# genetics-statistics/GEMMA

Hardware: AMD Instinct MI355X
Metric: SNPs/s (-lmm 1 Wald) at n=20k on 1/2/4/8 MI355X; U^T x HBM GB/s vs roofline (higher is better)
Workload: dtype f64 (U^T x as int8-digit MFMA products with exact int32 accumulation; every column of U scaled by its exact maximum and rounded to 6 base-256 digits = 2^-48 of that maximum -- fp64 keeps 2^-53 per entry; value_strict / strict_leg (7g6m: U^T x at or below the fp64 GEMM's own error) and fp64_gemm_path

## Files before the change

### gemma_amd/_lib.py

```python
import ctypes as C
import os

HERE = os.path.dirname(os.path.abspath(__file__))
LIB_PATH = os.path.join(HERE, "libgemma_hip.so")

SYMBOLS = [
    "gemma_hip_init", "gemma_hip_shutdown", "gemma_hip_abi_version", "gemma_hip_strerror",
    "gemma_hip_last_error", "gemma_hip_device_info", "gemma_hip_dgemm", "gemma_hip_dgemm_d",
    "gemma_hip_kin_begin", "gemma_hip_kin_add", "gemma_hip_kin_add_d", "gemma_hip_kin_end",
    "gemma_hip_kin_end_d", "gemma_hip_kin_loco_d", "gemma_hip_snp_qc", "gemma_hip_center", "gemma_hip_center_d", "gemma_hip_eigh",
    "gemma_hip_eigh_d", "gemma_hip_eigh_reserve", "gemma_hip_eigh_release", "gemma_hip_dbg_eigh_last", "gemma_hip_eigh_sharded_d", "gemma_hip_eigh_kept_K_sharded", "gemma_hip_calc_utx", "gemma_hip_lmm_setup", "gemma_hip_lmm_setup_d",
    "gemma_hip_lmm_null", "gemma_hip_lmm_set_indicator", "gemma_hip_lmm_batch", "gemma_hip_lmm_batch_d",
    "gemma_hip_lmm_assoc_d", "gemma_hip_lmm_finish", "gemma_hip_lm_setup", "gemma_hip_lm_batch", "gemma_hip_lm_batch_d",
    "gemma_hip_lm_finish", "gemma_hip_profile_enable",
    "gemma_hip_profile_read", "gemma_hip_dbg_tridiag", "gemma_hip_dbg_stedc", "gemma_hip_dbg_eigh2", "gemma_hip_dbg_utx", "gemma_hip_lmm_gene_batch", "gemma_hip_lmm_gene_batch_d", "gemma_hip_lmm_set_env",
    "gemma_hip_lmm_gxe_batch", "gemma_hip_lmm_gxe_batch_d",
    "gemma_hip_mvlmm_null", "gemma_hip_mvlmm_set", "gemma_hip_mvlmm_batch", "gemma_hip_mvlmm_batch_d",
    "gemma_hip_kin_end_keep", "gemma_hip_kept_K_get", "gemma_hip_eigh_kept_K", "gemma_hip_eigh_keep", "gemma_hip_kept_n",
    "gemma_hip_kept_bcast", "gemma_hip_kept_U_get", "gemma_hip_calc_utx_kept", "gemma_hip_lmm_setup_kept", "gemma_hip_kept_release",
    "gemma_hip_comm_unique_id", "gemma_hip_comm_init", "gemma_hip_comm_info", "gemma_hip_comm_bcast_d",
    "gemma_hip_comm_allreduce_sum_d", "gemma_hip_comm_finalize", "gemma_hip_comm_selftest", "gemma_hip_comm_stats", "gemma_hip_dbg_i8_digits", "gemma_hip_dbg_last_utx_path", "gemma_hip_lmm_batch_submit", "gemma_hip_lmm_batch_collect",
    "gemma_hip_dbg_last_utx_kernel", "gemma_hip_dbg_last_block_missing", "gemma_hip_dbg_last_i8_post", "gemma_hip_reload_env", "gemma_hip_lmm_batch_pipe_d", "gemma_hip_lmm_pipe_flush",
    "gemma_hip_spd_inverse", "gemma_hip_spd_inverse_d", "gemma_hip_vc_setup", "gemma_hip_vc_setup_d", "gemma_hip_vc_he",
    "gemma_hip_vc_reml", "gemma_hip_vc_timing", "gemma_hip_vc_release",
    "gemma_hip_ridge_setup", "gemma_hip_ridge_setup_d", "gemma_hip_ridge_setup_kept", "gemma_hip_ridge_set_r",
    "gemma_hip_ridge_set_indicator", "gemma_hip_ridge_batch", "gemma_hip_ridge_batch_d", "gemma_hip_ridge_finish",
    "gemma_hip_prdt_begin", "gemma_hip_prdt_add", "gemma_hip_prdt_add_d", "gemma_hip_prdt_add_bv", "gemma_hip_prdt_add_bv_d",
    "gemma_hip_prdt_end", "gemma_hip_prdt_kin",
    "gemma_hip_mqs_begin", "gemma_hip_mqs_add", "gemma_hip_mqs_add_d", "gemma_hip_mqs_end", "gemma_hip_mqs_get",
    "gemma_hip_mqs_S", "gemma_hip_mqs_S_d", "gemma_hip_mqs_release",
    "gemma_hip_cor_begin", "gemma_hip_cor_block", "gemma_hip_cor_block_d", "gemma_hip_cor_release",
    "gemma_hip_ci_begin", "gemma_hip_ci_xwz", "gemma_hip_ci_xwz_d", "gemma_hip_ci_xwz_end", "gemma_hip_ci_xtxwz",
    "gemma_hip_ci_xtxwz_d", "gemma_hip_ci_release",
]
COMM_ID_BYTES = 128

OK, EINVAL, ENODEV, ENOMEM, ERUNTIME, ESTATE, ENOCONV, ENOTPD = range(8)
GENO_F64_SNP_MAJOR, GENO_PLINK_2BIT, GENO_F64_IDV_MAJOR = 0, 1, 2
STAGE_INGEST, STAGE_UTX_GEMM, STAGE_ASSOC, STAGE_KIN_GEMM, STAGE_EIGH, STAGE_UTX_POST = range(6)


class SumStat(C.Structure):
    _fields_ = [(k, C.c_double) for k in
                ("beta", "se", "lambda_remle", "lambda_mle", "p_wald", "p_lrt", "p_score", "logl_H1")]

# ... 102 lines not shown
    L.gemma_hip_lm_batch.argtypes = [ci, vp, sz, sz, vp]
    L.gemma_hip_lm_batch_d.argtypes = [ci, vp, sz, sz, vp, vp]
    L.gemma_hip_profile_enable.argtypes = [ci]
    L.gemma_hip_profile_read.argtypes = [ci, C.POINTER(cd), C.POINTER(C.c_long), ci]
    L.gemma_hip_dbg_tridiag.argtypes = [dp, sz, dp, dp, dp, dp]
    L.gemma_hip_dbg_stedc.argtypes = [dp, dp, sz, dp, dp]
    L.gemma_hip_dbg_eigh2.argtypes = [dp, sz, dp, dp, dp]
    L.gemma_hip_dbg_utx.argtypes = [C.c_int, vp, sz, sz, C.c_int, dp]
    L.gemma_hip_kin_end_keep.argtypes = [C.POINTER(sz), ci]
    L.gemma_hip_kept_K_get.argtypes = [dp]
    L.gemma_hip_eigh_kept_K.argtypes = [vp, sz, dp, C.POINTER(cd)]
    L.gemma_hip_eigh_kept_K_sharded.argtypes = [vp, sz, dp, C.POINTER(cd)]
    L.gemma_hip_eigh_keep.argtypes = [dp, sz, dp, C.POINTER(cd)]
    L.gemma_hip_kept_n.argtypes = [C.POINTER(sz)]
    L.gemma_hip_kept_bcast.argtypes = [ci, C.POINTER(cd)]
    L.gemma_hip_kept_U_get.argtypes = [dp, dp]
    L.gemma_hip_calc_utx_kept.argtypes = [dp, sz, sz, dp]
    L.gemma_hip_lmm_setup_kept.argtypes = [C.POINTER(LmmCfg), dp, dp]
    L.gemma_hip_dbg_i8_digits.argtypes = [sz, C.POINTER(ci)]
    L.gemma_hip_dbg_last_utx_path.argtypes = [C.POINTER(ci)]
    L.gemma_hip_dbg_last_utx_kernel.argtypes = [C.POINTER(UtxKernelInfo)]
    L.gemma_hip_dbg_last_block_missing.argtypes = [C.POINTER(ci)]
    L.gemma_hip_dbg_last_i8_post.argtypes = [C.POINTER(C.c_long), C.POINTER(C.c_long), C.POINTER(ci)]
    L.gemma_hip_reload_env.argtypes = []
    L.gemma_hip_lmm_batch_pipe_d.argtypes = [ci, vp, sz, sz, vp, vp]
    L.gemma_hip_lmm_pipe_flush.argtypes = [vp]
    L.gemma_hip_lmm_batch_submit.argtypes = [ci, vp, sz, sz]
    L.gemma_hip_lmm_batch_collect.argtypes = [vp, C.POINTER(sz)]
    L.gemma_hip_comm_unique_id.argtypes = [vp]
    L.gemma_hip_comm_init.argtypes = [vp, ci, ci]
    L.gemma_hip_comm_info.argtypes = [C.POINTER(ci), C.POINTER(ci), C.POINTER(ci)]
    L.gemma_hip_comm_bcast_d.argtypes = [vp, sz, ci, vp]
    L.gemma_hip_comm_allreduce_sum_d.argtypes = [dp, sz, vp]
    L.gemma_hip_comm_selftest.argtypes = [vp]
    L.gemma_hip_comm_stats.argtypes = [C.POINTER(CommStats)]
    L.gemma_hip_spd_inverse.argtypes = [dp, sz, sz, C.POINTER(cd), C.POINTER(C.c_long)]
    L.gemma_hip_spd_inverse_d.argtypes = [dp, sz, sz, C.POINTER(cd), C.POINTER(C.c_long), vp]
    L.gemma_hip_vc_setup.argtypes = [sz, sz, C.POINTER(dp), sz, dp, sz, dp]
    L.gemma_hip_vc_setup_d.argtypes = [sz, sz, C.POINTER(dp), sz, dp, sz, dp]
    L.gemma_hip_vc_he.argtypes = [dp] * 6
    L.gemma_hip_vc_reml.argtypes = [ci] + [dp] * 6 + [C.POINTER(ci), C.POINTER(ci), C.POINTER(C.c_long), dp, sz]
    L.gemma_hip_vc_timing.argtypes = [dp]
    L.gemma_hip_vc_release.argtypes = []
    L.gemma_hip_ridge_setup.argtypes = [sz, dp, dp, dp, cd, sz, dp]
    L.gemma_hip_ridge_setup_d.argtypes = [sz, dp, sz, dp, dp, cd, sz, dp, vp]
    L.gemma_hip_ridge_setup_kept.argtypes = [dp, cd, sz, dp]
# ... 43 lines not shown
```

### gemma_amd/api.py

```python
import ctypes as C

import numpy as np

from . import _lib as L

SUMSTAT_DTYPE = np.dtype([(k, "f8") for k in
                          ("beta", "se", "lambda_remle", "lambda_mle", "p_wald", "p_lrt", "p_score",
                           "logl_H1")])
LMM_BATCH_SIZE = 20000
K_BATCH_SIZE = 20000


def _is_torch(x):
    return type(x).__module__.startswith("torch")


def _np64(a, name):
    if not isinstance(a, np.ndarray) or a.dtype != np.float64:
        raise TypeError("%s must be a float64 numpy array" % name)
    if a.ndim == 2 and a.strides[1] != 8:
        raise ValueError("%s must be row-major with unit column stride" % name)
    return a


# ... 39 lines not shown
    return ms.value, n.value


UTX_PATHS = {0: "fp64 MFMA GEMM", 1: "int8 digits, hard calls", 2: "int8 digits, dosages k/100", 3: "int8 digits, dosages k/1000"}


def last_utx_path():
    p = C.c_int()
    L.check(L.lib().gemma_hip_dbg_last_utx_path(C.byref(p)), "dbg_last_utx_path")
    return p.value


def last_utx_kernel():
    k = L.UtxKernelInfo()
    L.check(L.lib().gemma_hip_dbg_last_utx_kernel(C.byref(k)), "dbg_last_utx_kernel")
    return {"variant": k.variant, "rows": k.rows, "digits": k.digits, "fuse": k.fuse, "raster": k.raster,
            "launches": k.launches, "name": k.name.decode()}


def last_block_missing():
    a = C.c_int()
    L.check(L.lib().gemma_hip_dbg_last_block_missing(C.byref(a)), "dbg_last_block_missing")
    return a.value


def reload_env():
    L.check(L.lib().gemma_hip_reload_env(), "reload_env")


def fast_dgemm(TransA, TransB, alpha, A, B, beta, Cm):
    ta, tb = TransA.upper()[0], TransB.upper()[0]
    M, N = Cm.shape
    if ta not in "NT" or tb not in "NT":
        raise L.GemmaHipError(L.EINVAL, "fast_dgemm", "bad transpose flag")
    Ka = A.shape[0] if ta == "T" else A.shape[1]
    Ma = A.shape[1] if ta == "T" else A.shape[0]
    Kb = B.shape[1] if tb == "T" else B.shape[0]
    Nb = B.shape[0] if tb == "T" else B.shape[1]
    if Ma != M or Nb != N or Ka != Kb:
        raise L.GemmaHipError(L.EINVAL, "fast_dgemm", "Range error in dgemm")
    if _is_torch(Cm):
        rc = L.lib().gemma_hip_dgemm_d(ta.encode(), tb.encode(), M, N, Ka, alpha, C.c_void_p(A.data_ptr()),
                                       _tld(A), C.c_void_p(B.data_ptr()), _tld(B), beta,
                                       C.c_void_p(Cm.data_ptr()), _tld(Cm), _stream())
    else:
        _np64(A, "A"); _np64(B, "B"); _np64(Cm, "C")
# ... 1577 lines not shown
```

### gemma_amd/csrc/abi_kept_comm.inc.h

```cpp

namespace {
__global__ void subselect_kernel(const double *__restrict__ K, long ni_total, const int *__restrict__ map, long n,
                                 double *__restrict__ G) {
  const long c = (long)blockIdx.x * blockDim.x + threadIdx.x, r = blockIdx.y;
  if (c < n) G[r * n + c] = K[(long)map[r] * ni_total + map[c]];
}
double *kept_U() { return g_ctx.kept_UE.as<double>(); }
double *kept_eval() { return g_ctx.kept_UE.as<double>() + g_ctx.kept_n * g_ctx.kept_n; }
}

extern "C" int gemma_hip_kin_end_keep(size_t *ns_used, int allreduce) {
  NEED_INIT();
  if (!g_ctx.kin_active) return fail(GEMMA_HIP_ESTATE, "kin_end before kin_begin");
  const size_t n = g_ctx.kin_n;
  size_t ns = g_ctx.kin_ns;
  {
    int rc = kin_fold_i8(nullptr);
    if (rc) return rc;
  }
  if (allreduce && g_ctx.comm.active && g_ctx.comm.world > 1) {
    std::string err;
    if (g_ctx.comm.allreduce_sum(g_ctx.kin_K.as<double>(), n * n, nullptr, err)) return fail(GEMMA_HIP_ERUNTIME, "%s", err.c_str());
    if (g_ctx.scratch.reserve(16)) return fail(GEMMA_HIP_ENOMEM, "kin_end_keep: scratch");
    double cnt = (double)ns;
// ... 357 lines not shown
  if (g_ctx.i8_flag_at < 0 || !g_ctx.i8_rowsur.p) return GEMMA_HIP_OK;
  HIPCHK(hipDeviceSynchronize());
  HIPCHK(hipMemcpy(any, g_ctx.i8_rowsur.as<int>() + g_ctx.i8_flag_at, sizeof(int), hipMemcpyDeviceToHost));
  return GEMMA_HIP_OK;
}

extern "C" int gemma_hip_dbg_last_i8_post(long *short_rows, long *long_rows, int *epilogue) {
  NEED_INIT();
  if (!short_rows || !long_rows || !epilogue) return fail(GEMMA_HIP_EINVAL, "dbg_last_i8_post: null");
  *short_rows = *long_rows = -1;
  *epilogue = g_ctx.i8_last_epi;
  if (g_ctx.i8_rowsur_n <= 0 || !g_ctx.i8_rowsur.p) return GEMMA_HIP_OK;
  std::vector<int> cnt((size_t)g_ctx.i8_rowsur_n);
  HIPCHK(hipDeviceSynchronize());
  HIPCHK(hipMemcpy(cnt.data(), g_ctx.i8_rowsur.p, cnt.size() * sizeof(int), hipMemcpyDeviceToHost));
  *short_rows = *long_rows = 0;
  for (int c : cnt) {
    if (c > SUR_MAX) *long_rows += 1;
    else if (c > 0) *short_rows += 1;
  }
  return GEMMA_HIP_OK;
}

extern "C" int gemma_hip_reload_env(void) {
  const int digits0 = i8_digits_for(g_ctx.cfg.n), scale0 = g_ctx.knobs.i8_scale_max;
  g_ctx.knobs.load();
  if (g_ctx.i8_ready && (i8_digits_for(g_ctx.cfg.n) != digits0 || g_ctx.knobs.i8_scale_max != scale0))
    g_ctx.i8_ready = g_ctx.i8_colsum_ready = false;
  return GEMMA_HIP_OK;
}

extern "C" int gemma_hip_dbg_last_utx_path(int *path) {
  if (path) *path = g_ctx.last_utx_path;
  return GEMMA_HIP_OK;
}

extern "C" int gemma_hip_dbg_i8_digits(size_t n, int *digits) {
  if (digits) *digits = i8_digits_for(n);
  return GEMMA_HIP_OK;
}
```

### gemma_amd/csrc/abi_lmm_batch.inc.h

```cpp

static void xp_release() {
  Ctx::XPipe &x = g_ctx.xp;
  if (x.P) (void)hipStreamDestroy(x.P);
  if (x.Q) (void)hipStreamDestroy(x.Q);
  if (x.in_ready) (void)hipEventDestroy(x.in_ready);
  if (x.ingest_done) (void)hipEventDestroy(x.ingest_done);
  x.ingest_done = nullptr;
  x.ingest_valid = false;
  for (int i = 0; i < 2; ++i) {
    if (x.prod_done[i]) (void)hipEventDestroy(x.prod_done[i]);
    if (x.post_done[i]) (void)hipEventDestroy(x.post_done[i]);
    x.prod_done[i] = x.post_done[i] = nullptr;
    x.post_valid[i] = false;
  }
  x.P = x.Q = nullptr;
  x.in_ready = nullptr;
  x.count = 0;
  x.pending = false;
  x.cus = -1;
  x.shadow_A.release(); x.shadow_C.release(); x.shadow_mean.release(); x.shadow_rowsur.release();
}
static int xp_init() {
  Ctx::XPipe &x = g_ctx.xp;
  const int ncu = g_ctx.prop.multiProcessorCount;
// ... 127 lines not shown
  if (utx_i8_mode() != 1 || i8_sparse_mode() != 2) return 1;
  int q = g_ctx.knobs.overlap_chunks;
  q = std::max(1, std::min(q, 16));
  while (q > 1 && l < (size_t)q * 2 * S2_BM) --q;
  return q;
}
static int overlap_init() {
  if (g_ctx.ov_stream) return GEMMA_HIP_OK;
  HIPCHK(hipStreamCreateWithFlags(&g_ctx.ov_stream, hipStreamNonBlocking));
  for (auto &e : g_ctx.ov_ready) HIPCHK(hipEventCreateWithFlags(&e, hipEventDisableTiming));
  HIPCHK(hipEventCreateWithFlags(&g_ctx.ov_done, hipEventDisableTiming));
  return GEMMA_HIP_OK;
}
static int lmm_batch_plink_chunked(const void *geno, size_t l, size_t ld, gemma_sumstat *out_d, int chunks, hipStream_t s) {
  const size_t n = g_ctx.cfg.n;
  const size_t ldx = (n + 1) & ~(size_t)1;
  int rc = overlap_init();
  if (rc) return rc;
  if (g_ctx.UtX.reserve(l * ldx * 8)) return fail(GEMMA_HIP_ENOMEM, "lmm_batch: cannot allocate %zu bytes", l * ldx * 8);
  double *UtX = g_ctx.UtX.as<double>();
  g_ctx.last_utx_path = 1;
  I8Dims d;
  if ((rc = i8_begin(l, &d, s))) return rc;
  {
    ProfScope ps(GEMMA_STAGE_INGEST, s);
    IngestI8Args a;
    a.src = reinterpret_cast<const unsigned char *>(geno); a.ld = (long)ld; a.l = (long)l;
    a.idx_map = g_ctx.have_map ? g_ctx.idx_map.as<int>() : nullptr;
    a.n = (int)d.n; a.A = g_ctx.i8_A.as<int8_t>(); a.ldk = (long)d.ldk;
    a.mean = g_ctx.i8_mean.as<double>();
    hipLaunchKernelGGL(ingest_i8_kernel, dim3((unsigned)((l + 3) / 4)), dim3(256), 0, s, a);
    HIPCHK(hipGetLastError());
  }
  if ((rc = i8_meta_build(d, s))) return rc;
  const size_t per = round_up((l + chunks - 1) / chunks, (size_t)S2_BM);
  hipStream_t side = g_ctx.ov_stream;
  int c = 0;
  for (size_t row0 = 0; row0 < l; row0 += per, ++c) {
    const size_t rows = std::min(per, l - row0), rows_pad = std::min(per, d.lpad - row0);
    if ((rc = i8_gemm_rows(d, row0, rows_pad, s, UtX, ldx, rows))) break;
    if (hipEventRecord(g_ctx.ov_ready[c], s) != hipSuccess || hipStreamWaitEvent(side, g_ctx.ov_ready[c], 0) != hipSuccess) {
      rc = fail(GEMMA_HIP_ERUNTIME, "lmm_batch: %s", hipGetErrorString(hipGetLastError()));
      break;
    }
    if ((rc = i8_post_rows(l, d, row0, rows, UtX, ldx, side))) break;
    if ((rc = launch_assoc(UtX + row0 * ldx, rows, ldx, out_d + row0, side))) break;
  }
  (void)hipEventRecord(g_ctx.ov_done, side);
  (void)hipStreamWaitEvent(s, g_ctx.ov_done, 0);
  return rc;
}

static int xp_flush_fwd(hipStream_t s) { return xp_flush(s); }

extern "C" int gemma_hip_lmm_pipe_flush(void *stream) {
  NEED_INIT();
  return xp_flush(S(stream));
// ... 139 lines not shown
```

### gemma_amd/csrc/abi_utx.inc.h

```cpp

struct I8Dims {
  size_t n, ldk, npad, lpad, mrows;
  int fuse, digits, nplanes;
  int mdrop;
  int complete;
  int epi;
};
static const int *i8_anymiss(const I8Dims &d) { return d.complete ? g_ctx.i8_rowsur.as<int>() + d.lpad : nullptr; }
static int i8_sparse_mode() { return g_ctx.knobs.i8_sparse; }
static int i8_begin(size_t l, I8Dims *d, hipStream_t s, bool allow_epi = true) {
  int rc = i8_prepare_u(s);
  if (rc) return rc;
  d->n = g_ctx.cfg.n; d->ldk = g_ctx.i8_ldk; d->npad = g_ctx.i8_npad;
  d->lpad = round_up(l, i8_sparse_mode() == 2 ? (size_t)S2_BM : (size_t)I8P_BM); d->mrows = 2 * d->lpad;
  d->fuse = (g_ctx.knobs.i8_fuse && (double)d->n * 2.0 * 128.0 * 257.0 < 2147483648.0) ? 1 : 0;
  d->digits = g_ctx.i8_digits;
  d->nplanes = d->fuse ? (d->digits + 1) / 2 : d->digits;
  d->mdrop = (g_ctx.knobs.i8_mdrop && d->fuse && d->digits == 7 && i8_sparse_mode() == 2 && g_ctx.knobs.i8_rows == 16) ? 1 : 0;
  d->complete = (g_ctx.knobs.i8_complete && i8_sparse_mode() == 2 && g_ctx.knobs.i8_rows == 16) ? 1 : 0;
  d->epi = (allow_epi && g_ctx.knobs.i8_epilogue && i8_sparse_mode() == 2 && g_ctx.knobs.i8_rows == 16 && d->nplanes >= 2) ? 1 : 0;
  const size_t c_elems = (size_t)(d->nplanes - d->epi) * d->mrows * d->npad;
  if (g_ctx.i8_A.reserve(d->lpad * d->ldk) || g_ctx.i8_C.reserve(c_elems * 4) || g_ctx.i8_mean.reserve(l * 8))
    return fail(GEMMA_HIP_ENOMEM, "lmm_batch: int8 product buffers (%zu bytes)", d->lpad * d->ldk + c_elems * 4);
  if (d->lpad != l) HIPCHK(hipMemsetAsync(g_ctx.i8_A.p, 0, d->lpad * d->ldk, s));
  return GEMMA_HIP_OK;
}

static int i8_meta_build(const I8Dims &d, hipStream_t s) {
  const int mode = i8_sparse_mode();
  if (mode == 0) return GEMMA_HIP_OK;
  ProfScope ps(GEMMA_STAGE_INGEST, s);
  const size_t nk = d.ldk / I8_BK, total = d.lpad * nk * (mode == 2 ? 4 : 2);
  if (g_ctx.i8_meta.reserve(total * sizeof(uint4)) || g_ctx.i8_rowsur.reserve((d.lpad + 1) * sizeof(int)))
    return fail(GEMMA_HIP_ENOMEM, "lmm_batch: mask words of the sparse product");
  HIPCHK(hipMemsetAsync(g_ctx.i8_rowsur.p, 0, (d.lpad + 1) * sizeof(int), s));
  if (mode == 2)
    hipLaunchKernelGGL(sparse2_meta_kernel, dim3((unsigned)((total + 255) / 256)), dim3(256), 0, s, g_ctx.i8_A.as<int8_t>(),
                       (long)d.lpad, (long)d.ldk, g_ctx.i8_meta.as<uint4>(), g_ctx.i8_rowsur.as<int>(),
                       const_cast<int *>(i8_anymiss(d)));
  else
    hipLaunchKernelGGL(sparse_meta_kernel, dim3((unsigned)((total + 255) / 256)), dim3(256), 0, s, g_ctx.i8_A.as<int8_t>(),
                       (long)d.lpad, (long)d.ldk, g_ctx.i8_meta.as<uint4>(), g_ctx.i8_rowsur.as<int>());
  HIPCHK(hipGetLastError());
  g_ctx.i8_flag_at = (mode == 2 && d.complete) ? (long)d.lpad : -1;
  g_ctx.i8_rowsur_n = (long)d.lpad;
  return GEMMA_HIP_OK;
}

static int raster_for(int tiles_m, int tiles_n, int rb, hipStream_t s, const int2 **map_d) {
  Ctx::RasterSlot *lru = &g_ctx.i8_raster[0];
  for (auto &r : g_ctx.i8_raster) {
    if (r.tm == tiles_m && r.tn == tiles_n && r.rb == rb && r.dev.p) {
      r.used = ++g_ctx.i8_raster_clock;
      *map_d = r.dev.as<int2>();
      return GEMMA_HIP_OK;
    }
    if (r.used < lru->used) lru = &r;
  }
  if (lru->dev.p) HIPCHK(hipDeviceSynchronize());
  s2_build_raster(tiles_m, tiles_n, rb, lru->host);
  lru->tm = lru->tn = lru->rb = 0;
  if (lru->dev.reserve(lru->host.size() * sizeof(int2)))
    return fail(GEMMA_HIP_ENOMEM, "lmm_batch: tile raster (%zu bytes)", lru->host.size() * sizeof(int2));
  HIPCHK(hipMemcpyAsync(lru->dev.p, lru->host.data(), lru->host.size() * sizeof(int2), hipMemcpyHostToDevice, s));
  HIPCHK(hipStreamSynchronize(s));
  lru->tm = tiles_m; lru->tn = tiles_n; lru->rb = rb;
  lru->used = ++g_ctx.i8_raster_clock;
  *map_d = lru->dev.as<int2>();
// ... 140 lines not shown
    HIPCHK(hipGetLastError());
  }
  if (!d.epi) {
    hipLaunchKernelGGL(i8_combine_kernel, dim3((unsigned)((d.n + 1023) / 1024), (unsigned)std::min<size_t>(rows, 65535)),
                       dim3(256), 0, s,
                       g_ctx.i8_C.as<int>() + row0 * d.npad, (long)d.npad, (long)(d.mrows * d.npad), (long)d.lpad,
                       g_ctx.i8_mean.as<double>() + row0, g_ctx.i8_qinv.as<double>(), (long)rows, (long)d.n, UtX + row0 * ldx, (long)ldx,
                       1.0, d.fuse, d.digits, sur_cnt, sur_list, g_ctx.U, (long)d.n, d.mdrop, i8_anymiss(d));
    HIPCHK(hipGetLastError());
  } else if (sparse) {
    hipLaunchKernelGGL(i8_surplus_short_kernel, dim3((unsigned)rows), dim3(256), 0, s, sur_cnt, sur_list,
                       g_ctx.i8_mean.as<double>() + row0, g_ctx.U, (long)d.n, (long)d.n, (long)rows, UtX + row0 * ldx, (long)ldx);
    HIPCHK(hipGetLastError());
  }
  if (sparse) {
    hipLaunchKernelGGL(i8_surplus_fix_kernel, dim3((unsigned)rows), dim3(256), 0, s, Arow, (long)d.ldk,
                       g_ctx.i8_rowsur.as<int>() + row0, g_ctx.i8_mean.as<double>() + row0, g_ctx.U, (long)d.n, (long)d.n,
                       (long)rows, UtX + row0 * ldx, (long)ldx, SUR_MAX);
    HIPCHK(hipGetLastError());
  }
  return GEMMA_HIP_OK;
}

static int i8_product(size_t l, const I8Dims &d, double *UtX, size_t ldx, hipStream_t s) {
  int rc = i8_meta_build(d, s);
  if (!rc) rc = i8_gemm_rows(d, 0, d.lpad, s, UtX, ldx, l);
  if (!rc) rc = i8_post_rows(l, d, 0, l, UtX, ldx, s);
  return rc;
}

static int utx_plink_i8(const void *geno, size_t l, size_t ld, double *UtX, size_t ldx, hipStream_t s) {
  I8Dims d;
  int rc = i8_begin(l, &d, s);
  if (rc) return rc;
  {
    ProfScope ps(GEMMA_STAGE_INGEST, s);
    IngestI8Args a;
    a.src = reinterpret_cast<const unsigned char *>(geno); a.ld = (long)ld; a.l = (long)l;
    a.idx_map = g_ctx.have_map ? g_ctx.idx_map.as<int>() : nullptr;
    a.n = (int)d.n; a.A = g_ctx.i8_A.as<int8_t>(); a.ldk = (long)d.ldk;
    a.mean = g_ctx.i8_mean.as<double>();
    hipLaunchKernelGGL(ingest_i8_kernel, dim3((unsigned)((l + 3) / 4)), dim3(256), 0, s, a);
    HIPCHK(hipGetLastError());
  }
  return i8_product(l, d, UtX, ldx, s);
}

static bool dosage_i8_enabled() { return g_ctx.knobs.dosage_i8 != 0; }
static int utx_dosage_i8(const double *src, size_t l, size_t ld, bool nan_missing, bool two, bool have_m, const I8Dims &d,
                         double *UtX, size_t ldx, hipStream_t s) {
  const int np = (two ? 2 : 1) + (have_m ? 1 : 0);
  const size_t plane_a = d.lpad * d.ldk, plane_c = d.lpad * d.npad;
  if (g_ctx.i8_A.reserve((size_t)np * plane_a) || g_ctx.i8_C.reserve((size_t)np * d.digits * plane_c * 4) ||
      g_ctx.i8_colsum.reserve(d.n * 8))
    return fail(GEMMA_HIP_ENOMEM, "lmm_batch: dosage planes (%zu bytes)", (size_t)np * (plane_a + d.digits * plane_c * 4));
  int8_t *A0 = g_ctx.i8_A.as<int8_t>();
  {
    ProfScope ps(GEMMA_STAGE_INGEST, s);
    if (d.lpad != l) HIPCHK(hipMemsetAsync(A0, 0, (size_t)np * plane_a, s));
    PackDosageArgs a;
    a.src = src; a.ld = (long)ld; a.l = (long)l; a.n = (int)d.n; a.nan_missing = nan_missing ? 1 : 0; a.two = two ? 1 : 0;
    a.A0 = A0; a.A1 = two ? A0 + plane_a : nullptr; a.Am = have_m ? A0 + (size_t)(np - 1) * plane_a : nullptr;
    a.ldk = (long)d.ldk; a.mean = g_ctx.i8_mean.as<double>();
    hipLaunchKernelGGL(pack_dosage_kernel, dim3((unsigned)((l + 3) / 4)), dim3(256), 0, s, a);
    HIPCHK(hipGetLastError());
    if (!g_ctx.i8_colsum_ready) {
      hipLaunchKernelGGL(u_digit_colsum_kernel, dim3((unsigned)((d.n + 3) / 4)), dim3(256), 0, s, g_ctx.i8_Bt.as<int8_t>(),
                         (long)d.ldk, (long)(d.npad * d.ldk), g_ctx.i8_qinv.as<double>(), (long)d.n, d.digits,
// ... 100 lines not shown
```

### gemma_amd/csrc/gemma_hip.hip

```cpp
#include <hip/hip_runtime.h>

#include <cmath>
#include <cstdarg>
#include <cstdio>
#include <cstdlib>
#include <cstring>
#include <string>
#include <vector>

#include "../../include/gemma_hip.h"
#include "tu_common.h"
#include "dgemm_mfma.hip.h"
#include "eigh_tu.h"
#include "vc_tu.h"
#include "prdt_tu.h"
#include "mqs_tu.h"
#include "cor_tu.h"
#include "ingest.hip.h"
#include "lm_assoc.hip.h"
#include "lmm_assoc.hip.h"
#include "lmm_grid.hip.h"
#include "i8gemm.hip.h"
#include "i8gemm_sparse.hip.h"
#include "i8gemm_sparse2.hip.h"
// ... 6 lines not shown

using namespace gemma_hip;

namespace {

struct StageProf {
  std::vector<std::pair<hipEvent_t, hipEvent_t>> ev;
  double acc_ms = 0.0;
  long launches = 0;
};

struct Knobs {
  int utx_i8 = 1;
  int i8_digits = 0;
  int i8_sparse = 2;
  int i8_fuse = 1;
  int i8_gm = 0;
  int i8_raster = S2_DEFAULT_RASTER;
  int i8_rows = 16;
  int i8_scale_max = 1;
  int i8_mdrop = 0;
  int i8_complete = 1;
  int i8_epilogue = 1;
  int dosage_i8 = 1;
  int dosage_rows = 16;
  int overlap = 0;
  int overlap_chunks = 4;
  int table_v2 = 1;
  int table_pf = 0;
  int force_generic = 0;
  int assoc_variant = 44;
  int mvlmm_rt = 0;
  int pipe_cus = 64;
  int kin_i8 = 1, kin_upper = 1, kin_lists = 1, kin_lists_oom = 0;
  long long kin_list_cap = 0;
  static int geti(const char *name, int dflt) {
    const char *e = getenv(name);
    return (e && *e) ? atoi(e) : dflt;
  }
  void load() {
    utx_i8 = geti("GEMMA_HIP_UTX_I8", 1);
    const int dg = geti("GEMMA_HIP_I8_DIGITS", 0);
    i8_digits = (dg == 6 || dg == 7) ? dg : 0;
    const char *es = getenv("GEMMA_HIP_I8_SPARSE");
    i8_sparse = (es && es[0] >= '0' && es[0] <= '2') ? es[0] - '0' : 2;
    const char *ef = getenv("GEMMA_HIP_I8_FUSE");
    i8_fuse = (ef && ef[0] == '0') ? 0 : 1;
    i8_gm = geti("GEMMA_HIP_I8_GM", 0);
    i8_raster = geti("GEMMA_HIP_I8_RASTER", S2_DEFAULT_RASTER);
    i8_rows = geti("GEMMA_HIP_I8_ROWS", 16) == 32 ? 32 : 16;
    const char *esc = getenv("GEMMA_HIP_I8_SCALE");
    i8_scale_max = (esc && strcmp(esc, "pow2") == 0) ? 0 : 1;
    const char *efm = getenv("GEMMA_HIP_I8_FORM");
    i8_mdrop = (efm && strcmp(efm, "7g6m") == 0) ? 1 : 0;
    if (i8_mdrop) i8_digits = 7;
    const char *ecp = getenv("GEMMA_HIP_I8_COMPLETE");
    i8_complete = (ecp && ecp[0] == '0') ? 0 : 1;
    const char *eep = getenv("GEMMA_HIP_I8_EPILOGUE");
    i8_epilogue = (eep && eep[0] == '0') ? 0 : 1;
    const char *ed = getenv("GEMMA_HIP_UTX_DOSAGE_I8");
    dosage_i8 = (ed && ed[0] == '0') ? 0 : 1;
    dosage_rows = geti("GEMMA_HIP_DOSAGE_ROWS", 16) == 32 ? 32 : 16;
    const char *eo = getenv("GEMMA_HIP_OVERLAP");
    overlap = (eo && eo[0] == '1') ? 1 : 0;
    overlap_chunks = geti("GEMMA_HIP_OVERLAP_CHUNKS", 4);
    const char *et = getenv("GEMMA_HIP_TABLE_V2");
    table_v2 = (et && et[0] == '0') ? 0 : 1;
    const char *ep = getenv("GEMMA_HIP_TABLE_PF");
    table_pf = (ep && ep[0] == '1') ? 1 : 0;
    const char *eg = getenv("GEMMA_HIP_FORCE_GENERIC");
    force_generic = (eg && eg[0] == '1') ? 1 : 0;
    assoc_variant = geti("GEMMA_HIP_ASSOC_VARIANT", 44);
    const char *er = getenv("GEMMA_HIP_MVLMM_RT");
    mvlmm_rt = (er && er[0] == '1') ? 1 : 0;
    pipe_cus = geti("GEMMA_HIP_PIPE_CUS", 64);
    const char *k1 = getenv("GEMMA_HIP_KIN_I8"), *k2 = getenv("GEMMA_HIP_KIN_UPPER"), *k3 = getenv("GEMMA_HIP_KIN_LISTS");
    const char *k4 = getenv("GEMMA_HIP_KIN_LISTS_OOM"), *k5 = getenv("GEMMA_HIP_KIN_LIST_CAP");
    kin_i8 = (k1 && k1[0] == '0') ? 0 : 1;
    kin_upper = (k2 && k2[0] == '0') ? 0 : 1;
    kin_lists = (k3 && k3[0] == '0') ? 0 : 1;
    kin_lists_oom = (k4 && k4[0] == '1') ? 1 : 0;
    kin_list_cap = (k5 && *k5) ? atoll(k5) : 0;
// ... 55 lines not shown
  DevBuf table_P;
  DevBuf gxe_env, gxe_UtWt, gxe_Z, gxe_UtZ, gxe_flip;
  bool gxe_ready = false;
  double gxe_lnbeta = 0.0;
  DevBuf mv_Yt, mv_out;
  DevBuf mv_scratch;
  bool mv_ready = false, mv_gxe = false;
  size_t mv_d = 0;
  MvArgs mv_proto;
  DevBuf i8_Bt, i8_q, i8_qinv, i8_cmax, i8_A, i8_C, i8_mean;
  unsigned long long cheb_qmask = 0;
  struct RasterSlot {
    DevBuf dev;
    std::vector<int2> host;
    int tm = 0, tn = 0, rb = 0, xcds = 8;
    unsigned long long used = 0;
  } i8_raster[6];
  unsigned long long i8_raster_clock = 0;
  DevBuf i8_surlist;
  DevBuf i8_colsum;
  bool i8_colsum_ready = false;
  int last_utx_path = 0;
  gemma_utx_kernel_info last_utx_kernel = {};
  int i8_last_epi = -1;
  long i8_rowsur_n = 0;
  long i8_flag_at = -1;
  bool i8_ready = false;
  size_t i8_ldk = 0, i8_npad = 0;
  int i8_digits = I8_DIGITS;
  GridGeom grid_geom;
  int carry_flip = 0;
  AssocArgs assoc_proto;

  bool lm_active = false;
  LmArgs lm_proto;
  DevBuf lm_Wt, lm_y, lm_small;

  DevBuf scratch;

  struct PipeSlot {
    void *pin_in = nullptr, *pin_out = nullptr;
    size_t pin_in_cap = 0, pin_out_cap = 0;
    DevBuf dev_in, dev_out;
    hipEvent_t h2d = nullptr, done = nullptr;
    size_t l = 0;
    bool busy = false;
// ... 285 lines not shown
```

### gemma_amd/csrc/i8gemm_sparse2.hip.h

```cpp
#pragma once
#include <algorithm>
#include <vector>
#include "i8gemm_sparse.hip.h"

namespace gemma_hip {

constexpr int S2_BM = 256, S2_BN = 128;
constexpr int S2_AMB = 16384;
constexpr int S2_STAGE = 32768;
constexpr int S2_NST = 4;
#ifndef S2_ADVANCE
#define S2_ADVANCE 1
#endif
#ifndef S2_LOOPDMA
#define S2_LOOPDMA 1
#endif

struct Sparse2Args {
  const uint4 *AM;
  const int8_t *Bt;
  int *C;
  long ldk, ldc, strideB, strideC, m_row0;
  int tiles_m, tiles_n, nk, gm, fuse, digits;
  int plane0 = 0;
// ... 32 lines not shown
    const int8_t *src = base + 32 * (2 * p + h);
    unsigned idx = 0, bits = 0;
    int surplus = 0;
    for (int gq = 0; gq < 8; ++gq) {
      const unsigned word = *reinterpret_cast<const unsigned *>(src + 4 * gq);
      const unsigned m = (word >> 4) & 0x01010101u;
      const unsigned pat = (m | (m >> 7) | (m >> 14) | (m >> 21)) & 0xFu;
      const int cnt = __popc(pat);
      const int p0 = cnt >= 1 ? __ffs(pat) - 1 : 0;
      const unsigned rest = pat & (pat - 1);
      const int p1 = cnt >= 2 ? __ffs(rest) - 1 : (p0 == 3 ? 2 : 3);
      idx |= (unsigned)(p0 | (p1 << 2)) << (4 * gq);
      const int e0 = 2 * gq, e1 = 2 * gq + 1;
      bits |= (unsigned)(cnt >= 1) << (8 * (e0 & 3) + (e0 >> 2));
      bits |= (unsigned)(cnt >= 2) << (8 * (e1 & 3) + (e1 >> 2));
      surplus += cnt > 2 ? cnt - 2 : 0;
    }
    w[2] = idx;
    w[3] = bits;
    if (surplus) atomicAdd(row_surplus + row, surplus);
    if (anymiss && bits != 0 && *reinterpret_cast<volatile int *>(anymiss) == 0) *reinterpret_cast<volatile int *>(anymiss) = 1;
  }
  AM[id] = make_uint4(w[0], w[1], w[2], w[3]);
}

__device__ __forceinline__ i32x4 s2_unpack_g(int w) {
  i32x4 v;
  const unsigned u = (unsigned)w;
#pragma unroll
  for (int i = 0; i < 4; ++i) v[i] = (int)((u >> (2 * i)) & 0x03030303u);
  return v;
}
__device__ __forceinline__ i32x4 s2_expand(int bits) {
  i32x4 v;
  const unsigned u = (unsigned)bits;
#pragma unroll
  for (int i = 0; i < 4; ++i) v[i] = (int)((u >> i) & 0x01010101u);
  return v;
}

static inline void s2_build_raster(int tiles_m, int tiles_n, int rb, std::vector<int2> &map, int PR = 8) {
  const int NX = 8, PC = 32 / PR;
  if (rb != 1 && rb != 2 && rb != 4 && rb != 8) rb = 2;
  const int cbs = NX / rb;
  std::vector<std::vector<int2>> seq(NX);
  for (int band0 = 0, band = 0; band0 < tiles_m; band0 += rb * PR, ++band)
// ... 288 lines not shown
```

### include/gemma_hip.h

```cpp
#ifndef GEMMA_HIP_H
#define GEMMA_HIP_H

#include <stddef.h>

#ifdef __cplusplus
extern "C" {
#endif

#define GEMMA_HIP_ABI_VERSION 4

enum {
  GEMMA_HIP_OK = 0,
  GEMMA_HIP_EINVAL = 1,
  GEMMA_HIP_ENODEV = 2,
  GEMMA_HIP_ENOMEM = 3,
  GEMMA_HIP_ERUNTIME = 4,
  GEMMA_HIP_ESTATE = 5,
  GEMMA_HIP_ENOCONV = 6,
  GEMMA_HIP_ENOTPD = 7
};

typedef struct {
  double beta, se, lambda_remle, lambda_mle, p_wald, p_lrt, p_score, logl_H1;
} gemma_sumstat;
// ... 149 lines not shown
int gemma_hip_dbg_last_utx_path(int *path);
enum {
  GEMMA_UTX_KERNEL_DGEMM_F64 = 0,
  GEMMA_UTX_KERNEL_DENSE_I8 = 1,
  GEMMA_UTX_KERNEL_SPARSE_BYTES = 2,
  GEMMA_UTX_KERNEL_RECORDS_R32 = 3,
  GEMMA_UTX_KERNEL_RECORDS_R16 = 4,
  GEMMA_UTX_KERNEL_DOSAGE_I8 = 5,
  GEMMA_UTX_KERNEL_DOSAGE_I8_R16 = 6,
  GEMMA_UTX_KERNEL_COUNT = 7
};
typedef struct {
  int variant;
  int rows;
  int digits;
  int fuse;
  int raster;
  long launches;
  char name[64];
} gemma_utx_kernel_info;
int gemma_hip_dbg_last_utx_kernel(gemma_utx_kernel_info *info);
int gemma_hip_dbg_last_block_missing(int *any);
int gemma_hip_dbg_last_i8_post(long *short_rows, long *long_rows, int *epilogue);
int gemma_hip_reload_env(void);
int gemma_hip_dbg_i8_digits(size_t n, int *digits);

int gemma_hip_spd_inverse(double *A, size_t n, size_t lda, double *logdet, long *bad_pivot);
int gemma_hip_spd_inverse_d(double *A_d, size_t n, size_t lda, double *logdet, long *bad_pivot, void *stream);

int gemma_hip_vc_setup(size_t n, size_t n_vc, const double *const *K, size_t ldk, const double *W, size_t n_cvt, const double *y);
int gemma_hip_vc_setup_d(size_t n, size_t n_vc, const double *const *K_d, size_t ldk, const double *W, size_t n_cvt,
                         const double *y);
int gemma_hip_vc_he(double *sigma2, double *se_sigma2, double *pve, double *se_pve, double *pve_total, double *se_pve_total);
int gemma_hip_vc_reml(int noconstrain, double *sigma2, double *se_sigma2, double *pve, double *se_pve, double *pve_total,
                      double *se_pve_total, int *iterations, int *status, long *counts, double *iter_sigma2, size_t iter_cap);
int gemma_hip_vc_timing(double *t5);
int gemma_hip_vc_release(void);

int gemma_hip_ridge_setup(size_t n, const double *U, const double *eval, const double *Uty, double lambda, size_t ns_test,
                          double *bv_out);
int gemma_hip_ridge_setup_d(size_t n, const double *U_d, size_t ldu, const double *eval_d, const double *Uty_d, double lambda,
                            size_t ns_test, double *bv_out_d, void *stream);
int gemma_hip_ridge_setup_kept(const double *Uty, double lambda, size_t ns_test, double *bv_out);
int gemma_hip_ridge_set_r(size_t n, const double *r, double scale);
int gemma_hip_ridge_set_indicator(const int *indicator_idv, size_t ni_total);
int gemma_hip_ridge_batch(int geno_kind, const void *geno, size_t l, size_t ld, double *alpha_out);
// ... 43 lines not shown
```

Baseline: 370,300.

## Build sparse int8 product records directly from PLINK bytes during ingest

Adds an ingest kernel that reads PLINK 2-bit genotypes and writes the sparse-product records (packed genotype words, missing-index and bit masks, row means, surplus counts) in one pass. This skips the separate dense int8 expansion and meta-build pass for most rows. Only rows whose missing-count surplus is nonzero get the dense int8 row written. The padding memset is narrowed to the padded tail only. The path is on by default when sparse mode 2 applies, there is no index map and the input is aligned; otherwise the old byte ingest is kept. The cost is a more complex kernel with more bit manipulation per word, and a dense row A that is left unfilled for rows without surplus.

```diff
diff --git a/gemma_amd/_lib.py b/gemma_amd/_lib.py
--- a/gemma_amd/_lib.py
+++ b/gemma_amd/_lib.py
@@ -20,7 +20,7 @@
     "gemma_hip_kept_bcast", "gemma_hip_kept_U_get", "gemma_hip_calc_utx_kept", "gemma_hip_lmm_setup_kept", "gemma_hip_kept_release",
     "gemma_hip_comm_unique_id", "gemma_hip_comm_init", "gemma_hip_comm_info", "gemma_hip_comm_bcast_d",
     "gemma_hip_comm_allreduce_sum_d", "gemma_hip_comm_finalize", "gemma_hip_comm_selftest", "gemma_hip_comm_stats", "gemma_hip_dbg_i8_digits", "gemma_hip_dbg_last_utx_path", "gemma_hip_lmm_batch_submit", "gemma_hip_lmm_batch_collect",
-    "gemma_hip_dbg_last_utx_kernel", "gemma_hip_dbg_last_block_missing", "gemma_hip_dbg_last_i8_post", "gemma_hip_reload_env", "gemma_hip_lmm_batch_pipe_d", "gemma_hip_lmm_pipe_flush",
+    "gemma_hip_dbg_last_utx_kernel", "gemma_hip_dbg_last_block_missing", "gemma_hip_dbg_last_i8_post", "gemma_hip_dbg_last_i8_forms", "gemma_hip_reload_env", "gemma_hip_lmm_batch_pipe_d", "gemma_hip_lmm_pipe_flush",
     "gemma_hip_spd_inverse", "gemma_hip_spd_inverse_d", "gemma_hip_vc_setup", "gemma_hip_vc_setup_d", "gemma_hip_vc_he",
     "gemma_hip_vc_reml", "gemma_hip_vc_timing", "gemma_hip_vc_release",
     "gemma_hip_ridge_setup", "gemma_hip_ridge_setup_d", "gemma_hip_ridge_setup_kept", "gemma_hip_ridge_set_r",
@@ -169,6 +169,7 @@
     L.gemma_hip_dbg_last_utx_kernel.argtypes = [C.POINTER(UtxKernelInfo)]
     L.gemma_hip_dbg_last_block_missing.argtypes = [C.POINTER(ci)]
     L.gemma_hip_dbg_last_i8_post.argtypes = [C.POINTER(C.c_long), C.POINTER(C.c_long), C.POINTER(ci)]
+    L.gemma_hip_dbg_last_i8_forms.argtypes = [C.POINTER(ci)]
     L.gemma_hip_reload_env.argtypes = []
     L.gemma_hip_lmm_batch_pipe_d.argtypes = [ci, vp, sz, sz, vp, vp]
     L.gemma_hip_lmm_pipe_flush.argtypes = [vp]
diff --git a/gemma_amd/api.py b/gemma_amd/api.py
--- a/gemma_amd/api.py
+++ b/gemma_amd/api.py
@@ -85,6 +85,12 @@
     a = C.c_int()
     L.check(L.lib().gemma_hip_dbg_last_block_missing(C.byref(a)), "dbg_last_block_missing")
     return a.value
+
+
+def last_i8_forms():
+    a = C.c_int()
+    L.check(L.lib().gemma_hip_dbg_last_i8_forms(C.byref(a)), "dbg_last_i8_forms")
+    return {"records_ingest": a.value}
 
 
 def reload_env():
diff --git a/gemma_amd/csrc/abi_kept_comm.inc.h b/gemma_amd/csrc/abi_kept_comm.inc.h
--- a/gemma_amd/csrc/abi_kept_comm.inc.h
+++ b/gemma_amd/csrc/abi_kept_comm.inc.h
@@ -403,6 +403,12 @@
   return GEMMA_HIP_OK;
 }
 
+extern "C" int gemma_hip_dbg_last_i8_forms(int *records_ingest) {
+  if (!records_ingest) return fail(GEMMA_HIP_EINVAL, "dbg_last_i8_forms: null");
+  *records_ingest = g_ctx.i8_last_ingest_rec;
+  return GEMMA_HIP_OK;
+}
+
 extern "C" int gemma_hip_reload_env(void) {
   const int digits0 = i8_digits_for(g_ctx.cfg.n), scale0 = g_ctx.knobs.i8_scale_max;
   g_ctx.knobs.load();
diff --git a/gemma_amd/csrc/abi_lmm_batch.inc.h b/gemma_amd/csrc/abi_lmm_batch.inc.h
--- a/gemma_amd/csrc/abi_lmm_batch.inc.h
+++ b/gemma_amd/csrc/abi_lmm_batch.inc.h
@@ -173,17 +173,9 @@
   g_ctx.last_utx_path = 1;
   I8Dims d;
   if ((rc = i8_begin(l, &d, s))) return rc;
-  {
-    ProfScope ps(GEMMA_STAGE_INGEST, s);
-    IngestI8Args a;
-    a.src = reinterpret_cast<const unsigned char *>(geno); a.ld = (long)ld; a.l = (long)l;
-    a.idx_map = g_ctx.have_map ? g_ctx.idx_map.as<int>() : nullptr;
-    a.n = (int)d.n; a.A = g_ctx.i8_A.as<int8_t>(); a.ldk = (long)d.ldk;
-    a.mean = g_ctx.i8_mean.as<double>();
-    hipLaunchKernelGGL(ingest_i8_kernel, dim3((unsigned)((l + 3) / 4)), dim3(256), 0, s, a);
-    HIPCHK(hipGetLastError());
-  }
-  if ((rc = i8_meta_build(d, s))) return rc;
+  bool have_records = false;
+  if ((rc = i8_ingest_plink(geno, l, ld, d, s, &have_records))) return rc;
+  if (!have_records && (rc = i8_meta_build(d, s))) return rc;
   const size_t per = round_up((l + chunks - 1) / chunks, (size_t)S2_BM);
   hipStream_t side = g_ctx.ov_stream;
   int c = 0;
diff --git a/gemma_amd/csrc/abi_utx.inc.h b/gemma_amd/csrc/abi_utx.inc.h
--- a/gemma_amd/csrc/abi_utx.inc.h
+++ b/gemma_amd/csrc/abi_utx.inc.h
@@ -22,7 +22,7 @@
   const size_t c_elems = (size_t)(d->nplanes - d->epi) * d->mrows * d->npad;
   if (g_ctx.i8_A.reserve(d->lpad * d->ldk) || g_ctx.i8_C.reserve(c_elems * 4) || g_ctx.i8_mean.reserve(l * 8))
     return fail(GEMMA_HIP_ENOMEM, "lmm_batch: int8 product buffers (%zu bytes)", d->lpad * d->ldk + c_elems * 4);
-  if (d->lpad != l) HIPCHK(hipMemsetAsync(g_ctx.i8_A.p, 0, d->lpad * d->ldk, s));
+  if (d->lpad != l) HIPCHK(hipMemsetAsync(g_ctx.i8_A.as<int8_t>() + l * d->ldk, 0, (d->lpad - l) * d->ldk, s));
   return GEMMA_HIP_OK;
 }
 
@@ -44,6 +44,38 @@
   HIPCHK(hipGetLastError());
   g_ctx.i8_flag_at = (mode == 2 && d.complete) ? (long)d.lpad : -1;
   g_ctx.i8_rowsur_n = (long)d.lpad;
+  g_ctx.i8_last_ingest_rec = 0;
+  return GEMMA_HIP_OK;
+}
+
+static int i8_ingest_plink(const void *geno, size_t l, size_t ld, const I8Dims &d, hipStream_t s, bool *have_records) {
+  ProfScope ps(GEMMA_STAGE_INGEST, s);
+  *have_records = g_ctx.knobs.i8_ingest_rec && i8_sparse_mode() == 2 && !g_ctx.have_map &&
+                  (reinterpret_cast<uintptr_t>(geno) & 3) == 0 && (ld % 4 == 0 || l == 1);
+  if (!*have_records) {
+    IngestI8Args a;
+    a.src = reinterpret_cast<const unsigned char *>(geno); a.ld = (long)ld; a.l = (long)l;
+    a.idx_map = g_ctx.have_map ? g_ctx.idx_map.as<int>() : nullptr;
+    a.n = (int)d.n; a.A = g_ctx.i8_A.as<int8_t>(); a.ldk = (long)d.ldk;
+    a.mean = g_ctx.i8_mean.as<double>();
+    hipLaunchKernelGGL(ingest_i8_kernel, dim3((unsigned)((l + 3) / 4)), dim3(256), 0, s, a);
+    HIPCHK(hipGetLastError());
+    return GEMMA_HIP_OK;
+  }
+  const size_t nk = d.ldk / I8_BK;
+  if (g_ctx.i8_meta.reserve(d.lpad * nk * 4 * sizeof(uint4)) || g_ctx.i8_rowsur.reserve((d.lpad + 1) * sizeof(int)))
+    return fail(GEMMA_HIP_ENOMEM, "lmm_batch: records of the sparse product");
+  HIPCHK(hipMemsetAsync(g_ctx.i8_rowsur.p, 0, (d.lpad + 1) * sizeof(int), s));
+  IngestRecArgs a;
+  a.src = reinterpret_cast<const unsigned char *>(geno); a.ld = (long)ld; a.l = (long)l; a.lpad = (long)d.lpad;
+  a.n = (int)d.n; a.ldk = (long)d.ldk;
+  a.AM = g_ctx.i8_meta.as<uint4>(); a.A = g_ctx.i8_A.as<int8_t>(); a.mean = g_ctx.i8_mean.as<double>();
+  a.row_surplus = g_ctx.i8_rowsur.as<int>(); a.anymiss = const_cast<int *>(i8_anymiss(d));
+  hipLaunchKernelGGL(ingest_records_kernel, dim3((unsigned)((d.lpad + 3) / 4)), dim3(256), 0, s, a);
+  HIPCHK(hipGetLastError());
+  g_ctx.i8_flag_at = d.complete ? (long)d.lpad : -1;
+  g_ctx.i8_rowsur_n = (long)d.lpad;
+  g_ctx.i8_last_ingest_rec = 1;
   return GEMMA_HIP_OK;
 }
 
@@ -230,8 +262,8 @@
   return GEMMA_HIP_OK;
 }
 
-static int i8_product(size_t l, const I8Dims &d, double *UtX, size_t ldx, hipStream_t s) {
-  int rc = i8_meta_build(d, s);
+static int i8_product(size_t l, const I8Dims &d, double *UtX, size_t ldx, hipStream_t s, bool have_records = false) {
+  int rc = have_records ? GEMMA_HIP_OK : i8_meta_build(d, s);
   if (!rc) rc = i8_gemm_rows(d, 0, d.lpad, s, UtX, ldx, l);
   if (!rc) rc = i8_post_rows(l, d, 0, l, UtX, ldx, s);
   return rc;
@@ -241,17 +273,9 @@
   I8Dims d;
   int rc = i8_begin(l, &d, s);
   if (rc) return rc;
-  {
-    ProfScope ps(GEMMA_STAGE_INGEST, s);
-    IngestI8Args a;
-    a.src = reinterpret_cast<const unsigned char *>(geno); a.ld = (long)ld; a.l = (long)l;
-    a.idx_map = g_ctx.have_map ? g_ctx.idx_map.as<int>() : nullptr;
-    a.n = (int)d.n; a.A = g_ctx.i8_A.as<int8_t>(); a.ldk = (long)d.ldk;
-    a.mean = g_ctx.i8_mean.as<double>();
-    hipLaunchKernelGGL(ingest_i8_kernel, dim3((unsigned)((l + 3) / 4)), dim3(256), 0, s, a);
-    HIPCHK(hipGetLastError());
-  }
-  return i8_product(l, d, UtX, ldx, s);
+  bool have_records = false;
+  if ((rc = i8_ingest_plink(geno, l, ld, d, s, &have_records))) return rc;
+  return i8_product(l, d, UtX, ldx, s, have_records);
 }
 
 static bool dosage_i8_enabled() { return g_ctx.knobs.dosage_i8 != 0; }
diff --git a/gemma_amd/csrc/gemma_hip.hip b/gemma_amd/csrc/gemma_hip.hip
--- a/gemma_amd/csrc/gemma_hip.hip
+++ b/gemma_amd/csrc/gemma_hip.hip
@@ -52,6 +52,7 @@
   int i8_mdrop = 0;
   int i8_complete = 1;
   int i8_epilogue = 1;
+  int i8_ingest_rec = 1;
   int dosage_i8 = 1;
   int dosage_rows = 16;
   int overlap = 0;
@@ -88,6 +89,8 @@
     i8_complete = (ecp && ecp[0] == '0') ? 0 : 1;
     const char *eep = getenv("GEMMA_HIP_I8_EPILOGUE");
     i8_epilogue = (eep && eep[0] == '0') ? 0 : 1;
+    const char *eig = getenv("GEMMA_HIP_I8_INGEST");
+    i8_ingest_rec = (eig && strcmp(eig, "bytes") == 0) ? 0 : 1;
     const char *ed = getenv("GEMMA_HIP_UTX_DOSAGE_I8");
     dosage_i8 = (ed && ed[0] == '0') ? 0 : 1;
     dosage_rows = geti("GEMMA_HIP_DOSAGE_ROWS", 16) == 32 ? 32 : 16;
@@ -189,6 +192,7 @@
   bool i8_colsum_ready = false;
   int last_utx_path = 0;
   gemma_utx_kernel_info last_utx_kernel = {};
+  int i8_last_ingest_rec = -1;
   int i8_last_epi = -1;
   long i8_rowsur_n = 0;
   long i8_flag_at = -1;
diff --git a/gemma_amd/csrc/i8gemm_sparse2.hip.h b/gemma_amd/csrc/i8gemm_sparse2.hip.h
--- a/gemma_amd/csrc/i8gemm_sparse2.hip.h
+++ b/gemma_amd/csrc/i8gemm_sparse2.hip.h
@@ -78,6 +78,109 @@
     if (anymiss && bits != 0 && *reinterpret_cast<volatile int *>(anymiss) == 0) *reinterpret_cast<volatile int *>(anymiss) = 1;
   }
   AM[id] = make_uint4(w[0], w[1], w[2], w[3]);
+}
+
+struct IngestRecArgs {
+  const unsigned char *src;
+  long ld, l, lpad;
+  int n;
+  long ldk;
+  uint4 *AM;
+  int8_t *A;
+  double *mean;
+  int *row_surplus;
+  int *anymiss;
+};
+__device__ __forceinline__ unsigned s2_plink_word(const unsigned char *bs, long i0, int n) {
+  if (i0 >= n) return 0xFFFFFFFFu;
+  const long nbytes = ((long)n + 3) / 4;
+  unsigned w;
+  if (i0 / 4 + 4 <= nbytes) {
+    w = *reinterpret_cast<const unsigned *>(bs + i0 / 4);
+  } else {
+    w = 0u;
+    for (int b = 0; b < 4; ++b)
+      if (i0 / 4 + b < nbytes) w |= (unsigned)bs[i0 / 4 + b] << (8 * b);
+  }
+  const int nvalid = (n - i0 < 16) ? (int)(n - i0) : 16;
+  return nvalid < 16 ? (w | (0xFFFFFFFFu << (2 * nvalid))) : w;
+}
+__device__ __forceinline__ unsigned s2_plink_g2(unsigned w) {
+  const unsigned lo = w & 0x55555555u, hi = (w >> 1) & 0x55555555u;
+  const unsigned gf = (hi & ~lo) | ((~hi & ~lo & 0x55555555u) << 1);
+  unsigned g2 = 0;
+#pragma unroll
+  for (int i = 0; i < 4; ++i)
+#pragma unroll
+    for (int j = 0; j < 4; ++j) g2 |= ((gf >> (8 * i + 2 * j)) & 3u) << (8 * j + 2 * i);
+  return g2;
+}
+__global__ __launch_bounds__(256) void ingest_records_kernel(IngestRecArgs g) {
+  const int lane = threadIdx.x & 63;
+  const long s = (long)blockIdx.x * 4 + (threadIdx.x >> 6);
+  if (s >= g.lpad) return;
+  const long nk = g.ldk / I8_BK;
+  uint4 *out = g.AM + ((s / S2_BM) * nk * S2_BM + (s % S2_BM)) * 4;
+  if (s >= g.l) {
+    for (long u = lane; u < 2 * nk; u += 64) {
+      uint4 *o = out + (u >> 1) * (S2_BM * 4) + 2 * (u & 1);
+      o[0] = make_uint4(0u, 0u, 0u, 0u);
+      o[1] = make_uint4(0u, 0u, 0u, 0u);
+    }
+    return;
+  }
+  const unsigned char *bs = g.src + s * g.ld;
+  int itot = 0, imiss = 0, surplus = 0;
+  for (long u = lane; u < 2 * nk; u += 64) {
+    unsigned W[4], mf[4];
+#pragma unroll
+    for (int j = 0; j < 4; ++j) {
+      W[j] = s2_plink_word(bs, 16 * (4 * u + j), g.n);
+      const unsigned lo = W[j] & 0x55555555u, hi = (W[j] >> 1) & 0x55555555u;
+      mf[j] = lo & ~hi;
+      itot += __popc(hi & ~lo) + 2 * __popc(~hi & ~lo & 0x55555555u);
+      imiss += __popc(mf[j]);
+    }
+    uint4 rec[2];
+#pragma unroll
+    for (int h = 0; h < 2; ++h) {
+      unsigned idx = 0, bits = 0;
+#pragma unroll
+      for (int gq = 0; gq < 8; ++gq) {
+        const unsigned b = (mf[2 * h + (gq >> 2)] >> (8 * (gq & 3))) & 0x55u;
+        const unsigned pat = (b & 1u) | ((b >> 1) & 2u) | ((b >> 2) & 4u) | ((b >> 3) & 8u);
+        const int cnt = __popc(pat);
+        const int p0 = cnt >= 1 ? __ffs(pat) - 1 : 0;
+        const unsigned rest = pat & (pat - 1);
+        const int p1 = cnt >= 2 ? __ffs(rest) - 1 : (p0 == 3 ? 2 : 3);
+        idx |= (unsigned)(p0 | (p1 << 2)) << (4 * gq);
+        const int e0 = 2 * gq, e1 = 2 * gq + 1;
+        bits |= (unsigned)(cnt >= 1) << (8 * (e0 & 3) + (e0 >> 2));
+        bits |= (unsigned)(cnt >= 2) << (8 * (e1 & 3) + (e1 >> 2));
+        surplus += cnt > 2 ? cnt - 2 : 0;
+      }
+      rec[h] = make_uint4(s2_plink_g2(W[h]), s2_plink_g2(W[2 + h]), idx, bits);
+    }
+    uint4 *o = out + (u >> 1) * (S2_BM * 4) + 2 * (u & 1);
+    o[0] = rec[0];
+    o[1] = rec[1];
+  }
+  const double tot = wsum((double)itot), cnt = wsum((double)(0 - imiss)) + (double)g.n;
+  surplus = (int)wsum((double)surplus);
+  if (lane == 0) {
+    g.mean[s] = tot / cnt;
+    if (surplus) g.row_surplus[s] = surplus;
+    if (g.anymiss && cnt != (double)g.n && *reinterpret_cast<volatile int *>(g.anymiss) == 0) *reinterpret_cast<volatile int *>(g.anymiss) = 1;
+  }
+  if (surplus == 0) return;
+  int8_t *gr = g.A + s * g.ldk;
+  for (long k = lane; k < g.ldk / 16; k += 64) {
+    const unsigned w = s2_plink_word(bs, 16 * k, g.n);
+    unsigned o4[4] = {0u, 0u, 0u, 0u};
+#pragma unroll
+    for (int q = 0; q < 16; ++q) o4[q >> 2] |= ((0x00011002u >> (8 * ((w >> (2 * q)) & 3u))) & 0xFFu) << (8 * (q & 3));
+    *reinterpret_cast<uint4 *>(gr + 16 * k) = make_uint4(o4[0], o4[1], o4[2], o4[3]);
+  }
 }
 
 __device__ __forceinline__ i32x4 s2_unpack_g(int w) {
diff --git a/include/gemma_hip.h b/include/gemma_hip.h
--- a/include/gemma_hip.h
+++ b/include/gemma_hip.h
@@ -195,6 +195,7 @@
 int gemma_hip_dbg_last_utx_kernel(gemma_utx_kernel_info *info);
 int gemma_hip_dbg_last_block_missing(int *any);
 int gemma_hip_dbg_last_i8_post(long *short_rows, long *long_rows, int *epilogue);
+int gemma_hip_dbg_last_i8_forms(int *records_ingest);
 int gemma_hip_reload_env(void);
 int gemma_hip_dbg_i8_digits(size_t n, int *digits);
 
```

Result: no change. 372,500, median of 6 (+0.6%).
